# lpiccinelli-eth/UniDepth

Measured on NVIDIA H100. Metric: images/sec UniDepthV2.infer ViT-L/14 480x640, higher is better.
Workload: dtype f16 operands, f32 accumulate/residual

## Files before the change

include/udb.h:

```cpp
#ifndef UDB_H_
#define UDB_H_
#include <stddef.h>
#include <stdint.h>

#ifdef __cplusplus
extern "C" {
#endif

#define UDB_VERSION 1

int udb_version(void);

typedef struct udb_profile_entry_t {
  char name[48];
  float ms;
  double flops;
  double bytes;
} udb_profile_entry_t;
int udb_profile_begin(void* stream);
int udb_profile_end(udb_profile_entry_t* out, int32_t cap);
const char* udb_last_error(void);
int64_t udb_launch_count(void);

enum { UDB_A_MATRIX = 0, UDB_A_CONV3X3 = 1 };
// ... 16 lines not shown
  int32_t out_f32;
  void* out2;
  int32_t out2_leaky;
  int32_t act;
  int32_t store_mode;
  int64_t ldc;
  int32_t rows_per_group, group_stride, row_offset;
  int32_t resid_mod, resid_row_offset;
  int64_t ldr;
  int32_t ct_k, ct_cout, ct_h, ct_w, ct_pad;
  const float* head_w;
  float head_b, head_add;
  int32_t a_split_k;
  int32_t out_split;
  float* ln_stats_out;
  const float* ln_stats_in;
  const float* ln_c1;
  int32_t ln_parts, ln_part_cols;
  float ln_eps;
} udb_gemm_t;

int udb_gemm_f16(const udb_gemm_t* g, void* stream);
int udb_gemm_tma_epilogue_used(void);

typedef struct udb_conv_halo_t {
  const void* x;
  const void* w;
  const float* bias;
  int32_t B, H, W, C, cstride, coff, cout, act;
  void* out;
  int64_t ldc;
  const float* head_w;
  float head_b, head_add;
  float* head_out;
} udb_conv_halo_t;
int udb_conv3x3_halo_f16(const udb_conv_halo_t* c, void* stream);

typedef struct udb_attn_t {
  const void* q;
  const void* k;
  const void* v;
  void* out;
  int32_t B, heads, seq_q, seq_k, head_dim;
  int32_t ldq, ldk, ldv, ldo;
  int32_t q_col0, k_col0, v_col0, o_col0;
  float scale;
// ... 373 lines not shown
```

unidepth_b200/_cabi.py:

```python
from __future__ import annotations

import ctypes as C
import os

_HERE = os.path.dirname(os.path.abspath(__file__))
LIB_PATH = os.environ.get("UDB_LIB", os.path.join(_HERE, "libudb.so"))

A_MATRIX, A_CONV3X3 = 0, 1
ACT_NONE, ACT_GELU, ACT_LEAKY = 0, 1, 2
STORE_ROWS, STORE_CONVT, STORE_CONVTILE, STORE_HEAD = 0, 1, 2, 3
INTERP_BILINEAR, INTERP_BICUBIC = 0, 1
INTERP_MODES = {"bilinear": INTERP_BILINEAR, "bicubic": INTERP_BICUBIC}
CAM_NONE, CAM_PINHOLE, CAM_EUCM, CAM_SPHERICAL, CAM_OPENCV, CAM_FISHEYE624, CAM_MEI = range(7)
CAM_STRIDE = 20

vp, i32, i64, f32 = C.c_void_p, C.c_int32, C.c_int64, C.c_float


class Gemm(C.Structure):
    _fields_ = [
        ("a", vp), ("w", vp), ("M", i32), ("N", i32), ("K", i32), ("lda", i32), ("ldw", i32),
        ("a_mode", i32),
        ("conv_B", i32), ("conv_H", i32), ("conv_W", i32), ("conv_C", i32), ("conv_inH", i32),
        ("conv_inW", i32), ("conv_off", i32), ("conv_TH", i32), ("conv_TW", i32),
        ("conv_cstride", i32), ("conv_coff", i32),
        ("bias", vp), ("gamma", vp), ("resid", vp), ("resid_f32", i32), ("out", vp), ("out_f32", i32),
        ("out2", vp), ("out2_leaky", i32), ("act", i32), ("store_mode", i32), ("ldc", i64),
        ("rows_per_group", i32), ("group_stride", i32), ("row_offset", i32),
        ("resid_mod", i32), ("resid_row_offset", i32), ("ldr", i64),
        ("ct_k", i32), ("ct_cout", i32), ("ct_h", i32), ("ct_w", i32), ("ct_pad", i32),
        ("head_w", vp), ("head_b", f32), ("head_add", f32),
        ("a_split_k", i32), ("out_split", i32),
        ("ln_stats_out", vp), ("ln_stats_in", vp), ("ln_c1", vp), ("ln_parts", i32), ("ln_part_cols", i32), ("ln_eps", f32),
    ]


class ConvHalo(C.Structure):
    _fields_ = [
        ("x", vp), ("w", vp), ("bias", vp),
        ("B", i32), ("H", i32), ("W", i32), ("C", i32), ("cstride", i32), ("coff", i32), ("cout", i32), ("act", i32),
        ("out", vp), ("ldc", i64), ("head_w", vp), ("head_b", f32), ("head_add", f32), ("head_out", vp),
    ]


class Attn(C.Structure):
    _fields_ = [
        ("q", vp), ("k", vp), ("v", vp), ("out", vp),
        ("B", i32), ("heads", i32), ("seq_q", i32), ("seq_k", i32), ("head_dim", i32),
        ("ldq", i32), ("ldk", i32), ("ldv", i32), ("ldo", i32),
        ("q_col0", i32), ("k_col0", i32), ("v_col0", i32), ("o_col0", i32), ("scale", f32),
        ("split", i32), ("lo_off_q", i32), ("lo_off_k", i32), ("lo_off_v", i32), ("lo_off_o", i32),
    ]


class LayerNorm(C.Structure):
    _fields_ = [
        ("inp", vp), ("in_f32", i32), ("out", vp), ("out_f32", i32), ("weight", vp), ("bias", vp),
        ("rows", i32), ("dim", i32), ("ld_in", i64), ("ld_out", i64),
        ("rows_per_group", i32), ("group_stride", i32), ("row_offset", i32), ("eps", f32), ("dim_valid", i32),
# ... 138 lines not shown
METRIC_MAX_BLOCKS = 64
DM_AUC_BINS = 100
(DM_N, DM_D1, DM_D2, DM_D3, DM_TAU, DM_SQ, DM_SQLOG, DM_AREL, DM_SQREL, DM_LOG10, DM_LG, DM_LG2, DM_D1_SI, DM_TAU_SI,
 DM_AREL_SI, DM_PP, DM_P, DM_PG, DM_G, DM_AUC) = range(20)
DM_AREL_SSI, DM_D1_SSI, DM_TAU_SSI = DM_AUC + DM_AUC_BINS, DM_AUC + DM_AUC_BINS + 1, DM_AUC + DM_AUC_BINS + 2
DM_NACC = DM_TAU_SSI + 1
PM_MAX_THRESHOLDS = 1024


class ProfileEntry(C.Structure):
    _fields_ = [("name", C.c_char * 48), ("ms", f32), ("flops", C.c_double), ("bytes", C.c_double)]


DT_F16, DT_F32 = 0, 1

EXPORTS = {
    "udb_version": (i32, []),
    "udb_last_error": (C.c_char_p, []),
    "udb_launch_count": (i64, []),
    "udb_profile_begin": (i32, [vp]),
    "udb_profile_end": (i32, [C.POINTER(ProfileEntry), i32]),
    "udb_gemm_f16": (i32, [C.POINTER(Gemm), vp]),
    "udb_gemm_tma_epilogue_used": (i32, []),
    "udb_conv3x3_halo_f16": (i32, [C.POINTER(ConvHalo), vp]),
    "udb_attention_f16": (i32, [C.POINTER(Attn), vp]),
    "udb_layernorm": (i32, [C.POINTER(LayerNorm), vp]),
    "udb_preprocess_patchify": (i32, [C.POINTER(Preprocess), vp]),
    "udb_posembed_bicubic": (i32, [vp, i32, i32, vp, i32, i32, vp]),
    "udb_set_cls_rows": (i32, [vp, vp, vp, i32, i32, i32, vp]),
    "udb_set_cls_rows_ln": (i32, [vp, vp, vp, vp, vp, i32, i32, i32, i32, i32, vp]),
    "udb_small_linear_f32": (i32, [C.POINTER(SmallLinear), vp]),
    "udb_camera_attn4_f32": (i32, [vp, vp, vp, vp, i32, i32, i32, vp]),
    "udb_camera_intrinsics": (i32, [vp, i32, i32, i32, f32, i32, i32, vp, vp, vp, vp]),
    "udb_ray_embed": (i32, [C.POINTER(RayEmbed), vp]),
    "udb_upsample2x_nhwc_f16": (i32, [vp, vp, i32, i32, i32, i32, vp]),
    "udb_resize_ac_pad_nhwc_f16": (i32, [vp, vp, i32, i32, i32, i32, i32, i32, i32, vp]),
    "udb_reflect_pad1_nhwc_f16": (i32, [vp, vp, i32, i32, i32, i32, vp]),
    "udb_reflect_border_fill_nhwc_f16": (i32, [vp, i32, i32, i32, i32, vp]),
    "udb_postprocess": (i32, [C.POINTER(Postprocess), vp]),
    "udb_camera_adjust_k": (i32, [vp, i32, f32, i32, i32, vp, vp]),
    "udb_camera_rays": (i32, [i32, vp, i32, i32, i32, i32, i32, i32, i32, f32, vp, vp]),
    "udb_create": (i32, [C.POINTER(Config), C.POINTER(vp)]),
    "udb_destroy": (None, [vp]),
    "udb_set_weight": (i32, [vp, C.c_char_p, vp, C.POINTER(i64), i32, i32]),
    "udb_set_scalar": (i32, [vp, C.c_char_p, C.c_double]),
    "udb_geometry": (i32, [vp, i32, i32, i32, C.POINTER(Geometry)]),
# ... 82 lines not shown
```

unidepth_b200/csrc/gemm.cu:

```cuda
#include <stdlib.h>
#include <string.h>

#include "common.h"
#include "ptx.cuh"

namespace udb {

constexpr int BM = 128;
constexpr int BK = 64;
constexpr int kEpiWarps = 8;
constexpr int kTP = 36;
constexpr int kThreads = (kEpiWarps + 4) * 32;

struct GemmArgs {
  int M, N, K, num_kb;
  int tiles_m, tiles_n;
  int a_mode;
  int conv_B, conv_H, conv_W, conv_cpb , conv_off, conv_TH, conv_TW, conv_tx, conv_ty;
  const float* bias;
  const float* gamma;
  const void* resid;
  int resid_f32;
  void* out;
  int out_f32;
  __half* out2;
  int out2_leaky;
  int act;
  int store_mode;
  long long ldc, ldr;
  int rpg, gstride, roff;
  int resid_mod, resid_roff;
  int ct_k, ct_cout, ct_h, ct_w, ct_pad;
  int conv_coff;
  const float* head_w;
  float head_b, head_add;
  int a_wrap;
  int out_split;
  float* stats_out;
  const float* ln_stats;
  const float* ln_c1;
  int ln_parts, ln_part_cols;
  float ln_eps;
};

constexpr int kEpiBox = 64 * 32 * 4;

template <int BN, bool TMAE = false>
struct GemmCfg {
  static constexpr int kStages = TMAE ? (BN >= 192 ? 4 : (BN >= 128 ? 6 : 8))
                                      : (BN >= 256 ? 3 : (BN >= 192 ? 4 : (BN >= 128 ? 5 : 7)));
  static constexpr int kABytes = BM * BK * 2;
  static constexpr int kBBytes = BN * BK * 2;
  static constexpr int kStageBytes = kABytes + kBBytes;
  static constexpr int kStagingBytes = TMAE ? 2 * 2 * kEpiBox : kEpiWarps * (32 * kTP * 4 + 2 * 32 * 4);
  static constexpr int kSmemBytes = kStages * kStageBytes + kStagingBytes + 256 ;
  static_assert(kSmemBytes <= 232448, "shared memory per block");
  static_assert(2 * kStages + 4 <= 32, "barriers");
};

template <int N>
__device__ __forceinline__ void apply_act(const int act, float (&v)[N]) {
  if (act == UDB_ACT_GELU) {
#pragma unroll
    for (int j = 0; j < N; j += 2) gelu_erf_pair(v[j], v[j + 1]);
  } else if (act == UDB_ACT_LEAKY) {
#pragma unroll
    for (int j = 0; j < N; ++j) v[j] = leaky(v[j]);
  }
}

struct EpiWarp {
  float* T;
  float* Twg;
  uint32_t* roff_out;
  uint32_t* roff_res;
  int wg, wq, grp, lane, r_in_tile;
};

template <int BN, bool LNF>
__device__ __forceinline__ void epilogue_tile(const GemmArgs& p, const EpiWarp& w, const float (&acc)[BN / 2], const int mt,
                                              const int nt) {
  constexpr int kGroups = BN >= 64 ? 2 : 1;
  constexpr int kColsPerGrp = BN / kGroups;
  const int grp = w.grp, lane = w.lane, r_in_tile = w.r_in_tile;
  const bool active = grp < kGroups;
  float* T = w.T;
  uint32_t* roff_out = w.roff_out;
  uint32_t* roff_res = w.roff_res;
  bool valid = false;
  long long out_off = 0, res_off = 0;
  uint32_t vmask = 0;
  float ln_mean = 0.f, ln_rstd = 1.f;
  float st_pivot = 0.f, st_s1 = 0.f, st_s2 = 0.f;
  bool st_first = true;
  if (active) {

    const int m = mt * BM + r_in_tile;
    if (p.store_mode == UDB_STORE_CONVTILE || p.store_mode == UDB_STORE_HEAD) {
      const int per_img = p.conv_tx * p.conv_ty;
      const int b = mt / per_img;
      const int r = mt % per_img;
      const int y = (r / p.conv_tx) * p.conv_TH + r_in_tile / p.conv_TW;
      const int x = (r % p.conv_tx) * p.conv_TW + r_in_tile % p.conv_TW;
      valid = (b < p.conv_B) && (y < p.conv_H) && (x < p.conv_W);
// ... 30 lines not shown
        const float2 t = sp[q];
        m2 += t.y + (float)p.ln_part_cols * (t.x - ln_mean) * (t.x - ln_mean);
      }
      ln_rstd = rsqrtf(m2 / (float)(p.ln_parts * p.ln_part_cols) + p.ln_eps);
    }
  }
  const int frow = 16 * (w.wq & 1) + (lane >> 2), fcol = 2 * (lane & 3);
#pragma unroll
  for (int c = 0; c < kColsPerGrp; c += 32) {
    bar_sync(1 + w.wg, 128);
#pragma unroll
    for (int gi = 0; gi < kGroups; ++gi) {
      float* Tt = w.Twg + ((w.wq >> 1) | (gi << 1)) * 32 * kTP;
#pragma unroll
      for (int j = 0; j < 4; ++j) {
        const int f = ((gi * kColsPerGrp + c) / 8 + j) * 4;
        *reinterpret_cast<float2*>(Tt + frow * kTP + 8 * j + fcol) = make_float2(acc[f], acc[f + 1]);
        *reinterpret_cast<float2*>(Tt + (frow + 8) * kTP + 8 * j + fcol) = make_float2(acc[f + 2], acc[f + 3]);
      }
    }
    bar_sync(1 + w.wg, 128);
    if (!active) continue;
    const int col = grp * kColsPerGrp + c;
    const int n0 = nt * BN + col;
    float v[32];
#pragma unroll
    for (int j = 0; j < 32; j += 4) {
      const float4 t = *reinterpret_cast<const float4*>(T + lane * kTP + j);
      v[j] = t.x; v[j + 1] = t.y; v[j + 2] = t.z; v[j + 3] = t.w;
    }
    __syncwarp();
    if (n0 >= p.N) continue;
    if (LNF && p.ln_stats) {
      const float4* cp = reinterpret_cast<const float4*>(p.ln_c1 + n0);
      const float mr = ln_mean * ln_rstd;
#pragma unroll
      for (int j = 0; j < 8; ++j) {
        const float4 c4 = __ldg(cp + j);
        v[4 * j] = fmaf(v[4 * j], ln_rstd, -mr * c4.x);
        v[4 * j + 1] = fmaf(v[4 * j + 1], ln_rstd, -mr * c4.y);
        v[4 * j + 2] = fmaf(v[4 * j + 2], ln_rstd, -mr * c4.z);
        v[4 * j + 3] = fmaf(v[4 * j + 3], ln_rstd, -mr * c4.w);
      }
    }
    if (p.bias) {
      const float4* bp = reinterpret_cast<const float4*>(p.bias + n0);
#pragma unroll
// ... 117 lines not shown
    }
    if (p.out2) {
      if (p.out2_leaky) {
#pragma unroll
        for (int j = 0; j < 32; ++j) v[j] = leaky(v[j]);
        stage_rows(v);
      } else if (!p.out) {
        stage_rows(v);
      }
      __syncwarp();
      __half* op = p.out2 + c32 + l4;
      for_rows([&](int rr, bool ok) {
        const float4 t = *reinterpret_cast<const float4*>(T + rr * kTP + l4);
        if (ok) *reinterpret_cast<uint2*>(op + roff_out[rr]) = make_uint2(pack_half2(t.x, t.y), pack_half2(t.z, t.w));
      });
      __syncwarp();
    }
  }
  if (LNF && p.stats_out && active && valid && !st_first) {
    const float n = (float)kColsPerGrp;
    const float mean_p = st_pivot + st_s1 / n;
    const float m2_p = fmaxf(st_s2 - st_s1 * st_s1 / n, 0.f);
    const long long orow = out_off / p.ldc;
    reinterpret_cast<float2*>(p.stats_out)[orow * (p.tiles_n * kGroups) + nt * kGroups + grp] = make_float2(mean_p, m2_p);
  }
}

struct EpiTma {
  uint8_t* buf;
  uint64_t* full;
  uint64_t* empty;
  uint32_t chunk;
};

template <int BN>
__device__ __forceinline__ void epilogue_tile_tma(const GemmArgs& p, const CUtensorMap* tmC, EpiTma& e,
                                                  const float (&acc)[BN / 2], const int mt, const int nt, const int wg,
                                                  const int wq, const int lane) {
  const bool leader = wq == 0 && lane == 0;
  const int q = lane & 3, rr = lane >> 2;
  const bool has_res = p.resid != nullptr;
  const int row0 = mt * BM + 64 * wg;
#pragma unroll
  for (int c = 0; c < BN / 32; ++c, ++e.chunk) {
    const int b = e.chunk & 1;
    uint8_t* box = e.buf + (2 * b + wg) * kEpiBox;
    if (has_res) {
      mbar_wait(&e.full[b], (e.chunk >> 1) & 1);
    } else {
      if (leader) bulk_wait_read<1>();
      bar_sync(1 + wg, 128);
    }
    const int n0 = nt * BN + 32 * c;
    float v[16];
#pragma unroll
    for (int j = 0; j < 16; ++j) v[j] = acc[16 * c + j];
    if (p.bias) {
#pragma unroll
      for (int j = 0; j < 4; ++j) {
        const float2 b2 = __ldg(reinterpret_cast<const float2*>(p.bias + n0 + 8 * j + 2 * q));
        v[4 * j] += b2.x; v[4 * j + 1] += b2.y; v[4 * j + 2] += b2.x; v[4 * j + 3] += b2.y;
      }
    }
    apply_act(p.act, v);
    if (p.gamma) {
#pragma unroll
      for (int j = 0; j < 4; ++j) {
        const float2 g2 = __ldg(reinterpret_cast<const float2*>(p.gamma + n0 + 8 * j + 2 * q));
        v[4 * j] *= g2.x; v[4 * j + 1] *= g2.y; v[4 * j + 2] *= g2.x; v[4 * j + 3] *= g2.y;
      }
    }
    if (p.out_f32) {
#pragma unroll
      for (int j = 0; j < 4; ++j) {
#pragma unroll
        for (int h = 0; h < 2; ++h) {
// ... 11 lines not shown
#pragma unroll
      for (int j = 0; j < 4; ++j) {
#pragma unroll
        for (int h = 0; h < 2; ++h) {
          const int r = 16 * wq + rr + 8 * h;
          *reinterpret_cast<uint32_t*>(box + r * 64 + ((j ^ ((r >> 1) & 3)) << 4) + 4 * q) =
              pack_half2(v[4 * j + 2 * h], v[4 * j + 2 * h + 1]);
        }
      }
    }
    fence_proxy_async_smem();
    bar_sync(1 + wg, 128);
    if (leader) {
      if (row0 < p.M) tma_store_2d(tmC, box, n0, row0);
      bulk_commit();
      if (has_res) {
        bulk_wait_read<0>();
        mbar_arrive(&e.empty[b]);
      }
    }
  }
}

template <int BN, bool LNF, bool TMAE>
__global__ void __launch_bounds__(kThreads, 1)
gemm_f16_kernel(const __grid_constant__ CUtensorMap tmA, const __grid_constant__ CUtensorMap tmB,
                const __grid_constant__ CUtensorMap tmC, const __grid_constant__ CUtensorMap tmR, const GemmArgs p) {
  static_assert(!(TMAE && LNF), "the TMA epilogue carries no fused-LayerNorm code");
  using Cfg = GemmCfg<BN, TMAE>;
  constexpr int kStages = Cfg::kStages;
  extern __shared__ __align__(1024) uint8_t smem[];
  uint8_t* sA = smem;
  uint8_t* sB = smem + kStages * Cfg::kABytes;
  uint8_t* staging = smem + kStages * Cfg::kStageBytes;
  uint64_t* bars = reinterpret_cast<uint64_t*>(staging + Cfg::kStagingBytes);
  uint64_t* full_bar = bars;
  uint64_t* empty_bar = bars + kStages;
  uint64_t* epi_full = bars + 2 * kStages;
  uint64_t* epi_empty = epi_full + 2;

  const int warp = threadIdx.x >> 5;
  const int lane = threadIdx.x & 31;
  pdl_launch_dependents();

  if (threadIdx.x == 0) {
    if (smem_u32(smem) & 1023) __trap();
    prefetch_tmap(&tmA);
    prefetch_tmap(&tmB);
    for (int i = 0; i < kStages; ++i) {
      mbar_init(&full_bar[i], 1);
      mbar_init(&empty_bar[i], kEpiWarps);
    }
    if constexpr (TMAE) {
      prefetch_tmap(&tmC);
      if (p.resid) prefetch_tmap(&tmR);
      for (int i = 0; i < 2; ++i) {
        mbar_init(&epi_full[i], 1);
        mbar_init(&epi_empty[i], 2);
      }
    }
    fence_barrier_init();
  }
  __syncthreads();
  pdl_wait();

  const int num_tiles = p.tiles_m * p.tiles_n;

  if (warp >= kEpiWarps) {
    setmaxnreg_dec<40>();
    if constexpr (TMAE) {
      if (warp == kEpiWarps + 1 && p.resid) {
        const bool elected = elect_one();
        uint32_t chunk = 0;
        for (int tile = blockIdx.x; tile < num_tiles; tile += gridDim.x) {
          const int mt = tile / p.tiles_n;
          const int nt = tile % p.tiles_n;
          for (int c = 0; c < BN / 32; ++c, ++chunk) {
            const int b = chunk & 1;
            mbar_wait(&epi_empty[b], ((chunk >> 1) & 1) ^ 1);
            if (elected) {
              mbar_arrive_expect_tx(&epi_full[b], 2 * kEpiBox);
              tma_load_2d(staging + 2 * b * kEpiBox, &tmR, &epi_full[b], nt * BN + 32 * c, mt * BM);
            }
            __syncwarp();
          }
        }
      }
    }
    if (warp != kEpiWarps) return;
    const bool elected = elect_one();
    int stage = 0;
    uint32_t phase = 0;
    for (int tile = blockIdx.x; tile < num_tiles; tile += gridDim.x) {
      const int mt = tile / p.tiles_n;
      const int nt = tile % p.tiles_n;
      int cb = 0, cy = 0, cx = 0;
      if (p.a_mode == UDB_A_CONV3X3) {
        const int per_img = p.conv_tx * p.conv_ty;
        cb = mt / per_img;
        const int r = mt % per_img;
        cy = (r / p.conv_tx) * p.conv_TH + p.conv_off;
        cx = (r % p.conv_tx) * p.conv_TW + p.conv_off;
      }
      for (int kb = 0; kb < p.num_kb; ++kb) {
        mbar_wait(&empty_bar[stage], phase ^ 1);
        if (elected) {
          mbar_arrive_expect_tx(&full_bar[stage], Cfg::kStageBytes);
          if (p.a_mode == UDB_A_CONV3X3) {
            const int tap = kb / p.conv_cpb;
            const int c0 = p.conv_coff + (kb % p.conv_cpb) * BK;
            tma_load_4d(sA + stage * Cfg::kABytes, &tmA, &full_bar[stage], c0, cx + tap % 3, cy + tap / 3, cb);
          } else {
            int ka = kb * BK;
            if (p.a_wrap && ka >= p.a_wrap) ka -= p.a_wrap;
            tma_load_2d(sA + stage * Cfg::kABytes, &tmA, &full_bar[stage], ka, mt * BM);
          }
          tma_load_2d(sB + stage * Cfg::kBBytes, &tmB, &full_bar[stage], kb * BK, nt * BN);
        }
        __syncwarp();
        if (++stage == kStages) {
          stage = 0;
          phase ^= 1;
        }
      }
    }
  } else {
    setmaxnreg_inc<232>();
    const int wg = warp >> 2, wq = warp & 3;
    float* Twg = reinterpret_cast<float*>(staging) + wg * 4 * 32 * kTP;
    uint32_t* roff = reinterpret_cast<uint32_t*>(staging + kEpiWarps * 32 * kTP * 4) + warp * 64;
    const EpiWarp ctx{Twg + wq * 32 * kTP, Twg, roff, roff + 32, wg, wq, wq >> 1, lane, 64 * wg + 32 * (wq & 1) + lane};
    EpiTma etma{staging, epi_full, epi_empty, 0};
    float acc[BN / 2];
#pragma unroll
    for (int i = 0; i < BN / 2; ++i) acc[i] = 0.f;
    int stage = 0;
    uint32_t phase = 0;
    for (int tile = blockIdx.x; tile < num_tiles; tile += gridDim.x) {
      const int mt = tile / p.tiles_n;
      const int nt = tile % p.tiles_n;
      int prev = -1;
      for (int kb = 0; kb < p.num_kb; ++kb) {
        mbar_wait(&full_bar[stage], phase);
        const uint64_t da = gmma_desc_sw128(smem_u32(sA + stage * Cfg::kABytes + wg * 64 * 128), 16, 1024);
        const uint64_t db = gmma_desc_sw128(smem_u32(sB + stage * Cfg::kBBytes), 16, 1024);
        wgmma_fence();
#pragma unroll
        for (int k = 0; k < BK / 16; ++k) WgmmaSS<BN>::run(acc, da + 2 * k, db + 2 * k, (kb | k) != 0 ? 1u : 0u);
        wgmma_commit();
        wgmma_wait<1>();
        if (prev >= 0 && lane == 0) mbar_arrive(&empty_bar[prev]);
        prev = stage;
        if (++stage == kStages) {
          stage = 0;
          phase ^= 1;
        }
      }
      wgmma_wait<0>();
      wgmma_fence_regs(acc);
      if (prev >= 0 && lane == 0) mbar_arrive(&empty_bar[prev]);
      if constexpr (TMAE) epilogue_tile_tma<BN>(p, &tmC, etma, acc, mt, nt, wg, wq, lane);
      else epilogue_tile<BN, LNF>(p, ctx, acc, mt, nt);
    }
    if constexpr (TMAE) {
      if (wq == 0 && lane == 0) bulk_wait<0>();
    }
  }
}

template <int BN, bool LNF, bool TMAE>
static int launch_gemm(const CUtensorMap& tmA, const CUtensorMap& tmB, const CUtensorMap& tmC, const CUtensorMap& tmR,
                       const GemmArgs& a, cudaStream_t st) {
  using Cfg = GemmCfg<BN, TMAE>;
  static std::atomic<uint64_t> attr_mask{0};
  if (first_on_device(attr_mask)) {
    cudaError_t e = cudaFuncSetAttribute(gemm_f16_kernel<BN, LNF, TMAE>, cudaFuncAttributeMaxDynamicSharedMemorySize,
                                         Cfg::kSmemBytes);
    if (e != cudaSuccess) {
      set_error("gemm: cudaFuncSetAttribute(%d B smem): %s", Cfg::kSmemBytes, cudaGetErrorString(e));
      return 1;
    }
  }
  const int tiles = a.tiles_m * a.tiles_n;
  const int grid = tiles < num_sms() ? tiles : num_sms();
  cudaError_t e = launch_ex(gemm_f16_kernel<BN, LNF, TMAE>, dim3(grid), dim3(kThreads), Cfg::kSmemBytes, st, 1, tmA, tmB, tmC,
                            tmR, a);
  if (e != cudaSuccess) {
    set_error("gemm_f16_kernel launch: %s", cudaGetErrorString(e));
    return 1;
  }
  return check_launch("gemm_f16_kernel");
}

static bool aligned(const void* p, uintptr_t bytes) { return (reinterpret_cast<uintptr_t>(p) & (bytes - 1)) == 0; }

static int check_gemm_layout(const udb_gemm_t* g) {
  const int sm = g->store_mode;
  if (g->M < 1 || g->N < 1 || g->K < 1) { set_error("udb_gemm_f16: M=%d N=%d K=%d must be >= 1", g->M, g->N, g->K); return 1; }
  if (sm < UDB_STORE_ROWS || sm > UDB_STORE_HEAD) { set_error("udb_gemm_f16: unknown store_mode %d", sm); return 1; }
  const long long ldr = g->ldr > 0 ? g->ldr : g->ldc;
  if (sm == UDB_STORE_HEAD) {
    if (!g->out || !g->out_f32 || !aligned(g->out, 4)) { set_error("udb_gemm_f16: HEAD store needs a 4-byte aligned f32 `out`"); return 1; }
    if (!g->head_w || !aligned(g->head_w, 16)) { set_error("udb_gemm_f16: `head_w` must be non-null and 16-byte aligned"); return 1; }
  } else {
    if (g->out && !aligned(g->out, g->out_f32 ? 16 : 8)) {
      set_error("udb_gemm_f16: `out` %p must be %d-byte aligned", g->out, g->out_f32 ? 16 : 8); return 1;
    }
    if (g->out2 && !aligned(g->out2, 8)) { set_error("udb_gemm_f16: `out2` %p must be 8-byte aligned", g->out2); return 1; }
    if (g->resid && !aligned(g->resid, g->resid_f32 ? 16 : 8)) {
// ... 58 lines not shown

  if (g->a_mode == UDB_A_CONV3X3) {
    const int pad = g->conv_off == 0 ? 2 : (g->conv_off == -1 ? 0 : -1);
    if (pad < 0) { set_error("udb_gemm_f16: `conv_off`=%d must be 0 (prepadded) or -1 (zero padding)", g->conv_off); return 1; }
    if (g->conv_inH != g->conv_H + pad || g->conv_inW != g->conv_W + pad) {
      set_error("udb_gemm_f16: `conv_inH`x`conv_inW` = %dx%d must be %dx%d for conv_off %d", g->conv_inH, g->conv_inW, g->conv_H + pad,
                g->conv_W + pad, g->conv_off);
      return 1;
    }
  }
  return 0;
}

static bool tma_epilogue_ok(const udb_gemm_t* g) {
  const char* env = getenv("UDB_GEMM_TMA_EPILOGUE");
  if (env && atoi(env) == 0) return false;
  if (g->store_mode != UDB_STORE_ROWS || g->a_mode != UDB_A_MATRIX || g->rows_per_group > 0 || g->resid_mod > 0) return false;
  if (g->out_split || g->out2 || g->ln_stats_out || g->ln_stats_in || !g->out) return false;
  if (!aligned(g->out, 16) || (g->ldc * (g->out_f32 ? 4 : 2)) % 16) return false;
  const long long ldr = g->ldr > 0 ? g->ldr : g->ldc;
  return !g->resid || (g->resid_f32 && g->out_f32 && aligned(g->resid, 16) && (ldr * 4) % 16 == 0);
}

static thread_local int g_last_tma_epilogue = 0;

}

extern "C" int udb_gemm_tma_epilogue_used(void) { return udb::g_last_tma_epilogue; }

extern "C" int udb_gemm_f16(const udb_gemm_t* g, void* stream) {
  using namespace udb;
  if (!g || !g->a || !g->w) { set_error("udb_gemm_f16: null operand"); return 1; }
  if (g->N % 32 != 0) { set_error("udb_gemm_f16: N=%d must be a multiple of 32", g->N); return 1; }
  if (check_gemm_layout(g)) return 1;
  GemmArgs a{};
  a.M = g->M; a.N = g->N; a.K = g->K;
  a.num_kb = (g->K + BK - 1) / BK;
  a.a_mode = g->a_mode;
  a.bias = g->bias; a.gamma = g->gamma; a.resid = g->resid; a.resid_f32 = g->resid_f32;
  a.out = g->out; a.out_f32 = g->out_f32; a.out2 = reinterpret_cast<__half*>(g->out2); a.out2_leaky = g->out2_leaky;
  a.act = g->act; a.store_mode = g->store_mode;
  a.ldc = g->ldc; a.ldr = g->ldr > 0 ? g->ldr : g->ldc;
  a.rpg = g->rows_per_group; a.gstride = g->group_stride; a.roff = g->row_offset;
  a.resid_mod = g->resid_mod; a.resid_roff = g->resid_row_offset;
  a.ct_k = g->ct_k; a.ct_cout = g->ct_cout; a.ct_h = g->ct_h; a.ct_w = g->ct_w; a.ct_pad = g->ct_pad;
  a.conv_coff = g->conv_coff;
  a.head_w = g->head_w; a.head_b = g->head_b; a.head_add = g->head_add;
  a.a_wrap = 0;
  a.out_split = g->out_split;
  if (g->a_split_k > 0) {
    if (g->a_mode != UDB_A_MATRIX || g->a_split_k % BK || g->K != 3 * g->a_split_k || g->lda < 2 * g->a_split_k) {
      set_error("udb_gemm_f16: split operands need a_mode MATRIX, K1 %% 64 == 0, K == 3*K1, lda >= 2*K1 (K1=%d K=%d lda=%d)",
                g->a_split_k, g->K, g->lda);
      return 1;
    }
    a.a_wrap = 2 * g->a_split_k;
  }
  a.stats_out = g->ln_stats_out; a.ln_stats = g->ln_stats_in; a.ln_c1 = g->ln_c1; a.ln_eps = g->ln_eps;
  a.ln_parts = g->ln_parts; a.ln_part_cols = g->ln_part_cols;
  if ((g->ln_stats_out || g->ln_stats_in) && g->store_mode != UDB_STORE_ROWS) {
    set_error("udb_gemm_f16: fused LayerNorm statistics need the ROWS store"); return 1;
  }
  if (g->ln_stats_in && (!g->ln_c1 || g->ln_parts <= 0 || g->ln_part_cols <= 0 || g->rows_per_group > 0)) {
    set_error("udb_gemm_f16: ln_stats_in needs ln_c1, ln_parts, ln_part_cols and an identity row map"); return 1;
  }
  if (g->out_split && (g->out_f32 || !g->out || g->store_mode != UDB_STORE_ROWS)) {
    set_error("udb_gemm_f16: out_split needs an f16 `out` with the ROWS store"); return 1;
  }

  int bn;
  if (g->store_mode == UDB_STORE_HEAD) {
    if (g->N != 32) { set_error("udb_gemm_f16: HEAD store needs N == 32"); return 1; }
    bn = 32;
  } else if (g->N % 256 == 0) bn = 256;
  else if (g->N % 192 == 0) bn = 192;
  else if (g->N % 128 == 0) bn = 128;
  else if (g->N % 64 == 0) bn = 64;
  else bn = 32;
  if (g->store_mode == UDB_STORE_CONVT && (g->ct_cout % 32) != 0) {
    set_error("udb_gemm_f16: CONVT needs Cout %% 32 == 0"); return 1;
  }
  a.tiles_n = (g->N + bn - 1) / bn;
  if (g->ln_stats_out) {
    const int groups = bn >= 64 ? 2 : 1;
    if (g->N % bn || g->ln_parts != a.tiles_n * groups || g->ln_part_cols != bn / groups) {
      set_error("udb_gemm_f16: ln_stats_out with N=%d runs as %d parts of %d columns (caller said %d x %d)", g->N, a.tiles_n * groups,
                bn / groups, g->ln_parts, g->ln_part_cols);
      return 1;
    }
  }

  CUtensorMap tmA, tmB;
  if (g->a_mode == UDB_A_CONV3X3) {
    if (g->conv_C % BK != 0 || g->K != 9 * g->conv_C) {
      set_error("udb_gemm_f16: conv3x3 needs C %% 64 == 0 and K == 9*C (C=%d K=%d)", g->conv_C, g->K);
      return 1;
    }
    if (g->store_mode != UDB_STORE_CONVTILE && g->store_mode != UDB_STORE_HEAD) {
      set_error("udb_gemm_f16: conv3x3 operand needs a CONVTILE or HEAD store"); return 1;
    }
    const int TH = g->conv_TH > 0 ? g->conv_TH : 8, TW = g->conv_TW > 0 ? g->conv_TW : 16;
    if (TH * TW != BM) { set_error("udb_gemm_f16: conv tile %dx%d != 128 pixels", TH, TW); return 1; }
    a.conv_B = g->conv_B; a.conv_H = g->conv_H; a.conv_W = g->conv_W; a.conv_cpb = g->conv_C / BK; a.conv_off = g->conv_off;
    a.conv_TH = TH; a.conv_TW = TW;
    a.conv_tx = (g->conv_W + TW - 1) / TW; a.conv_ty = (g->conv_H + TH - 1) / TH;
    a.tiles_m = g->conv_B * a.conv_tx * a.conv_ty;
    a.M = a.tiles_m * BM;
    const uint64_t cs = g->conv_cstride > 0 ? g->conv_cstride : g->conv_C;
    if ((uint64_t)g->conv_coff + g->conv_C > cs || (g->conv_coff % 8)) {
      set_error("udb_gemm_f16: bad conv channel slice (off %d, C %d, stride %d)", g->conv_coff, g->conv_C, (int)cs);
      return 1;
    }
    const uint64_t dims[4] = {cs, (uint64_t)g->conv_inW, (uint64_t)g->conv_inH, (uint64_t)g->conv_B};
    const uint64_t str[3] = {cs * 2, (uint64_t)g->conv_inW * cs * 2, (uint64_t)g->conv_inH * g->conv_inW * cs * 2};
    const uint32_t box[4] = {(uint32_t)BK, (uint32_t)TW, (uint32_t)TH, 1};
    if (make_tmap_f16(&tmA, g->a, 4, dims, str, box, true)) return 1;
  } else {
    a.tiles_m = (g->M + BM - 1) / BM;
    if (g->store_mode == UDB_STORE_CONVTILE || g->store_mode == UDB_STORE_HEAD) {
      set_error("udb_gemm_f16: tile store modes need a_mode == CONV3X3"); return 1;
    }
    const uint64_t dims[2] = {(uint64_t)(g->a_split_k > 0 ? 2 * g->a_split_k : g->K), (uint64_t)g->M};
    const uint64_t str[1] = {(uint64_t)g->lda * 2};
    const uint32_t box[2] = {(uint32_t)BK, (uint32_t)BM};
    if (make_tmap_f16(&tmA, g->a, 2, dims, str, box, true)) return 1;
  }
  {
    const uint64_t dims[2] = {(uint64_t)g->K, (uint64_t)g->N};
    const uint64_t str[1] = {(uint64_t)g->ldw * 2};
    const uint32_t box[2] = {(uint32_t)BK, (uint32_t)bn};
    if (make_tmap_f16(&tmB, g->w, 2, dims, str, box, true)) return 1;
  }
  const bool tmae = tma_epilogue_ok(g);
  CUtensorMap tmC, tmR;
  memset(&tmC, 0, sizeof(tmC));
  memset(&tmR, 0, sizeof(tmR));
  if (tmae) {
    const uint64_t dims[2] = {(uint64_t)g->N, (uint64_t)g->M};
    const uint64_t str_c[1] = {(uint64_t)g->ldc * (g->out_f32 ? 4 : 2)};
    const uint32_t box_c[2] = {32, 64};
    if (make_tmap(&tmC, g->out, 2, dims, str_c, box_c, g->out_f32 ? CU_TENSOR_MAP_DATA_TYPE_FLOAT32 : CU_TENSOR_MAP_DATA_TYPE_FLOAT16,
                  g->out_f32 ? CU_TENSOR_MAP_SWIZZLE_128B : CU_TENSOR_MAP_SWIZZLE_64B))
      return 1;
    if (g->resid) {
      const uint64_t str_r[1] = {(uint64_t)a.ldr * 4};
      const uint32_t box_r[2] = {32, BM};
      if (make_tmap(&tmR, g->resid, 2, dims, str_r, box_r, CU_TENSOR_MAP_DATA_TYPE_FLOAT32, CU_TENSOR_MAP_SWIZZLE_128B)) return 1;
    }
  }
  g_last_tma_epilogue = tmae ? 1 : 0;
  cudaStream_t st = reinterpret_cast<cudaStream_t>(stream);
  note_work(2.0 * a.M * (double)g->N * g->K,
            2.0 * ((double)a.M * (g->a_mode == UDB_A_CONV3X3 ? g->conv_C : (g->a_split_k ? 2 * g->a_split_k : g->K)) + (double)g->N * g->K) +
                (double)a.M * g->N * ((g->out ? (g->out_f32 ? 4 : 2) : 0) + (g->out2 ? 2 : 0) + (g->resid ? (g->resid_f32 ? 4 : 2) : 0)));
  const bool lnf = g->ln_stats_out || g->ln_stats_in;
  if (lnf) {
    switch (bn) {
      case 256: return launch_gemm<256, true, false>(tmA, tmB, tmC, tmR, a, st);
      case 192: return launch_gemm<192, true, false>(tmA, tmB, tmC, tmR, a, st);
      case 128: return launch_gemm<128, true, false>(tmA, tmB, tmC, tmR, a, st);
      case 64: return launch_gemm<64, true, false>(tmA, tmB, tmC, tmR, a, st);
      default: return launch_gemm<32, true, false>(tmA, tmB, tmC, tmR, a, st);
    }
  }
  if (tmae) {
    switch (bn) {
      case 256: return launch_gemm<256, false, true>(tmA, tmB, tmC, tmR, a, st);
      case 192: return launch_gemm<192, false, true>(tmA, tmB, tmC, tmR, a, st);
      case 128: return launch_gemm<128, false, true>(tmA, tmB, tmC, tmR, a, st);
      case 64: return launch_gemm<64, false, true>(tmA, tmB, tmC, tmR, a, st);
      default: return launch_gemm<32, false, true>(tmA, tmB, tmC, tmR, a, st);
    }
  }
  switch (bn) {
    case 256: return launch_gemm<256, false, false>(tmA, tmB, tmC, tmR, a, st);
    case 192: return launch_gemm<192, false, false>(tmA, tmB, tmC, tmR, a, st);
    case 128: return launch_gemm<128, false, false>(tmA, tmB, tmC, tmR, a, st);
    case 64: return launch_gemm<64, false, false>(tmA, tmB, tmC, tmR, a, st);
    default: return launch_gemm<32, false, false>(tmA, tmB, tmC, tmR, a, st);
  }
}
```

Baseline: 222.4.

## Split last-wave GEMM tiles into narrow N units to balance persistent scheduling

```diff
diff --git a/include/udb.h b/include/udb.h
--- a/include/udb.h
+++ b/include/udb.h
@@ -62,6 +62,13 @@
 
 int udb_gemm_f16(const udb_gemm_t* g, void* stream);
 int udb_gemm_tma_epilogue_used(void);
+
+typedef struct udb_gemm_plan_t {
+  int32_t bn, tiles_m, tiles_n, grid, full, units, width;
+} udb_gemm_plan_t;
+int udb_gemm_plan(const udb_gemm_t* g, int32_t num_sms, udb_gemm_plan_t* plan);
+int udb_gemm_plan_unit(const udb_gemm_plan_t* plan, int32_t unit, int32_t* mt, int32_t* n0, int32_t* width);
+int udb_gemm_last_units(int32_t* full, int32_t* narrow, int32_t* width);
 
 typedef struct udb_conv_halo_t {
   const void* x;
diff --git a/unidepth_b200/_cabi.py b/unidepth_b200/_cabi.py
--- a/unidepth_b200/_cabi.py
+++ b/unidepth_b200/_cabi.py
@@ -35,6 +35,10 @@
     ]
 
 
+class GemmPlan(C.Structure):
+    _fields_ = [("bn", i32), ("tiles_m", i32), ("tiles_n", i32), ("grid", i32), ("full", i32), ("units", i32), ("width", i32)]
+
+
 class ConvHalo(C.Structure):
     _fields_ = [
         ("x", vp), ("w", vp), ("bias", vp),
@@ -219,6 +223,9 @@
     "udb_profile_end": (i32, [C.POINTER(ProfileEntry), i32]),
     "udb_gemm_f16": (i32, [C.POINTER(Gemm), vp]),
     "udb_gemm_tma_epilogue_used": (i32, []),
+    "udb_gemm_plan": (i32, [C.POINTER(Gemm), i32, C.POINTER(GemmPlan)]),
+    "udb_gemm_plan_unit": (i32, [C.POINTER(GemmPlan), i32, C.POINTER(i32), C.POINTER(i32), C.POINTER(i32)]),
+    "udb_gemm_last_units": (i32, [C.POINTER(i32), C.POINTER(i32), C.POINTER(i32)]),
     "udb_conv3x3_halo_f16": (i32, [C.POINTER(ConvHalo), vp]),
     "udb_attention_f16": (i32, [C.POINTER(Attn), vp]),
     "udb_layernorm": (i32, [C.POINTER(LayerNorm), vp]),
diff --git a/unidepth_b200/csrc/gemm.cu b/unidepth_b200/csrc/gemm.cu
--- a/unidepth_b200/csrc/gemm.cu
+++ b/unidepth_b200/csrc/gemm.cu
@@ -1,5 +1,7 @@
 #include <stdlib.h>
 #include <string.h>
+
+#include <type_traits>
 
 #include "common.h"
 #include "ptx.cuh"
@@ -41,7 +43,19 @@
   const float* ln_c1;
   int ln_parts, ln_part_cols;
   float ln_eps;
+  int units, units_full;
 };
+
+__host__ __device__ constexpr int tail_width(int bn) { return bn >= 128 ? 64 : 32; }
+
+struct GemmUnit {
+  int mt, n0, width;
+};
+__host__ __device__ __forceinline__ GemmUnit gemm_unit(int u, int tiles_n, int bn, int full, int w) {
+  if (u < full) return {u / tiles_n, (u % tiles_n) * bn, bn};
+  const int per = bn / w, r = u - full, tile = full + r / per;
+  return {tile / tiles_n, (tile % tiles_n) * bn + (r % per) * w, w};
+}
 
 constexpr int kEpiBox = 64 * 32 * 4;
 
@@ -79,7 +93,7 @@
 
 template <int BN, bool LNF>
 __device__ __forceinline__ void epilogue_tile(const GemmArgs& p, const EpiWarp& w, const float (&acc)[BN / 2], const int mt,
-                                              const int nt) {
+                                              const int nb) {
   constexpr int kGroups = BN >= 64 ? 2 : 1;
   constexpr int kColsPerGrp = BN / kGroups;
   const int grp = w.grp, lane = w.lane, r_in_tile = w.r_in_tile;
@@ -156,7 +170,7 @@
     bar_sync(1 + w.wg, 128);
     if (!active) continue;
     const int col = grp * kColsPerGrp + c;
-    const int n0 = nt * BN + col;
+    const int n0 = nb + col;
     float v[32];
 #pragma unroll
     for (int j = 0; j < 32; j += 4) {
@@ -320,7 +334,7 @@
     const float mean_p = st_pivot + st_s1 / n;
     const float m2_p = fmaxf(st_s2 - st_s1 * st_s1 / n, 0.f);
     const long long orow = out_off / p.ldc;
-    reinterpret_cast<float2*>(p.stats_out)[orow * (p.tiles_n * kGroups) + nt * kGroups + grp] = make_float2(mean_p, m2_p);
+    reinterpret_cast<float2*>(p.stats_out)[orow * (p.tiles_n * kGroups) + (nb / BN) * kGroups + grp] = make_float2(mean_p, m2_p);
   }
 }
 
@@ -333,7 +347,7 @@
 
 template <int BN>
 __device__ __forceinline__ void epilogue_tile_tma(const GemmArgs& p, const CUtensorMap* tmC, EpiTma& e,
-                                                  const float (&acc)[BN / 2], const int mt, const int nt, const int wg,
+                                                  const float (&acc)[BN / 2], const int mt, const int nb, const int wg,
                                                   const int wq, const int lane) {
   const bool leader = wq == 0 && lane == 0;
   const int q = lane & 3, rr = lane >> 2;
@@ -349,7 +363,7 @@
       if (leader) bulk_wait_read<1>();
       bar_sync(1 + wg, 128);
     }
-    const int n0 = nt * BN + 32 * c;
+    const int n0 = nb + 32 * c;
     float v[16];
 #pragma unroll
     for (int j = 0; j < 16; ++j) v[j] = acc[16 * c + j];
@@ -407,16 +421,25 @@
   }
 }
 
-template <int BN, bool LNF, bool TMAE>
+template <int BN, bool LNF, bool TMAE, bool SPLIT>
 __global__ void __launch_bounds__(kThreads, 1)
 gemm_f16_kernel(const __grid_constant__ CUtensorMap tmA, const __grid_constant__ CUtensorMap tmB,
-                const __grid_constant__ CUtensorMap tmC, const __grid_constant__ CUtensorMap tmR, const GemmArgs p) {
+                const __grid_constant__ CUtensorMap tmBn, const __grid_constant__ CUtensorMap tmC,
+                const __grid_constant__ CUtensorMap tmR, const GemmArgs p) {
   static_assert(!(TMAE && LNF), "the TMA epilogue carries no fused-LayerNorm code");
   using Cfg = GemmCfg<BN, TMAE>;
   constexpr int kStages = Cfg::kStages;
+  static_assert(!SPLIT || (!LNF && tail_width(BN) < BN), "no narrow units for this instantiation");
+  constexpr int kTW = SPLIT ? tail_width(BN) : BN;
+  constexpr int kNBBytes = kTW * BK * 2;
+  constexpr int kNK = SPLIT && Cfg::kBBytes >= Cfg::kABytes + 2 * kNBBytes ? 2 : 1;
   extern __shared__ __align__(1024) uint8_t smem[];
   uint8_t* sA = smem;
   uint8_t* sB = smem + kStages * Cfg::kABytes;
+  auto stage_a = [&](int s, int i) { return i == 0 ? sA + s * Cfg::kABytes : sB + s * Cfg::kBBytes; };
+  auto stage_b = [&](int s, int i, bool narrow) {
+    return sB + s * Cfg::kBBytes + (kNK == 2 && narrow ? Cfg::kABytes + i * kNBBytes : 0);
+  };
   uint8_t* staging = smem + kStages * Cfg::kStageBytes;
   uint64_t* bars = reinterpret_cast<uint64_t*>(staging + Cfg::kStagingBytes);
   uint64_t* full_bar = bars;
@@ -432,6 +455,7 @@
     if (smem_u32(smem) & 1023) __trap();
     prefetch_tmap(&tmA);
     prefetch_tmap(&tmB);
+    if (SPLIT) prefetch_tmap(&tmBn);
     for (int i = 0; i < kStages; ++i) {
       mbar_init(&full_bar[i], 1);
       mbar_init(&empty_bar[i], kEpiWarps);
@@ -449,23 +473,20 @@
   __syncthreads();
   pdl_wait();
 
-  const int num_tiles = p.tiles_m * p.tiles_n;
-
   if (warp >= kEpiWarps) {
     setmaxnreg_dec<40>();
     if constexpr (TMAE) {
       if (warp == kEpiWarps + 1 && p.resid) {
         const bool elected = elect_one();
         uint32_t chunk = 0;
-        for (int tile = blockIdx.x; tile < num_tiles; tile += gridDim.x) {
-          const int mt = tile / p.tiles_n;
-          const int nt = tile % p.tiles_n;
-          for (int c = 0; c < BN / 32; ++c, ++chunk) {
+        for (int u = blockIdx.x; u < p.units; u += gridDim.x) {
+          const GemmUnit t = gemm_unit(u, p.tiles_n, BN, p.units_full, kTW);
+          for (int c = 0; c < t.width / 32; ++c, ++chunk) {
             const int b = chunk & 1;
             mbar_wait(&epi_empty[b], ((chunk >> 1) & 1) ^ 1);
             if (elected) {
               mbar_arrive_expect_tx(&epi_full[b], 2 * kEpiBox);
-              tma_load_2d(staging + 2 * b * kEpiBox, &tmR, &epi_full[b], nt * BN + 32 * c, mt * BM);
+              tma_load_2d(staging + 2 * b * kEpiBox, &tmR, &epi_full[b], t.n0 + 32 * c, t.mt * BM);
             }
             __syncwarp();
           }
@@ -476,9 +497,12 @@
     const bool elected = elect_one();
     int stage = 0;
     uint32_t phase = 0;
-    for (int tile = blockIdx.x; tile < num_tiles; tile += gridDim.x) {
-      const int mt = tile / p.tiles_n;
-      const int nt = tile % p.tiles_n;
+    for (int u = blockIdx.x; u < p.units; u += gridDim.x) {
+      const GemmUnit t = gemm_unit(u, p.tiles_n, BN, p.units_full, kTW);
+      const int mt = t.mt;
+      const bool narrow = SPLIT && t.width != BN;
+      const CUtensorMap* tmW = narrow ? &tmBn : &tmB;
+      const int kpb = narrow ? kNK : 1;
       int cb = 0, cy = 0, cx = 0;
       if (p.a_mode == UDB_A_CONV3X3) {
         const int per_img = p.conv_tx * p.conv_ty;
@@ -487,20 +511,24 @@
         cy = (r / p.conv_tx) * p.conv_TH + p.conv_off;
         cx = (r % p.conv_tx) * p.conv_TW + p.conv_off;
       }
-      for (int kb = 0; kb < p.num_kb; ++kb) {
+      for (int kb0 = 0; kb0 < p.num_kb; kb0 += kpb) {
         mbar_wait(&empty_bar[stage], phase ^ 1);
         if (elected) {
-          mbar_arrive_expect_tx(&full_bar[stage], Cfg::kStageBytes);
-          if (p.a_mode == UDB_A_CONV3X3) {
-            const int tap = kb / p.conv_cpb;
-            const int c0 = p.conv_coff + (kb % p.conv_cpb) * BK;
-            tma_load_4d(sA + stage * Cfg::kABytes, &tmA, &full_bar[stage], c0, cx + tap % 3, cy + tap / 3, cb);
-          } else {
-            int ka = kb * BK;
-            if (p.a_wrap && ka >= p.a_wrap) ka -= p.a_wrap;
-            tma_load_2d(sA + stage * Cfg::kABytes, &tmA, &full_bar[stage], ka, mt * BM);
+          const int nk = kpb == 1 || p.num_kb - kb0 >= kpb ? kpb : p.num_kb - kb0;
+          mbar_arrive_expect_tx(&full_bar[stage], nk * (Cfg::kABytes + t.width * BK * 2));
+          for (int i = 0; i < nk; ++i) {
+            const int kb = kb0 + i;
+            if (p.a_mode == UDB_A_CONV3X3) {
+              const int tap = kb / p.conv_cpb;
+              const int c0 = p.conv_coff + (kb % p.conv_cpb) * BK;
+              tma_load_4d(stage_a(stage, i), &tmA, &full_bar[stage], c0, cx + tap % 3, cy + tap / 3, cb);
+            } else {
+              int ka = kb * BK;
+              if (p.a_wrap && ka >= p.a_wrap) ka -= p.a_wrap;
+              tma_load_2d(stage_a(stage, i), &tmA, &full_bar[stage], ka, mt * BM);
+            }
+            tma_load_2d(stage_b(stage, i, narrow), tmW, &full_bar[stage], kb * BK, t.n0);
           }
-          tma_load_2d(sB + stage * Cfg::kBBytes, &tmB, &full_bar[stage], kb * BK, nt * BN);
         }
         __syncwarp();
         if (++stage == kStages) {
@@ -521,18 +549,24 @@
     for (int i = 0; i < BN / 2; ++i) acc[i] = 0.f;
     int stage = 0;
     uint32_t phase = 0;
-    for (int tile = blockIdx.x; tile < num_tiles; tile += gridDim.x) {
-      const int mt = tile / p.tiles_n;
-      const int nt = tile % p.tiles_n;
+    auto run_unit = [&](auto width, const GemmUnit& t) {
+      constexpr int W = decltype(width)::value;
+      float(&accw)[W / 2] = *reinterpret_cast<float(*)[W / 2]>(acc);
+      constexpr int KPB = W != BN ? kNK : 1;
       int prev = -1;
-      for (int kb = 0; kb < p.num_kb; ++kb) {
+      for (int kb0 = 0; kb0 < p.num_kb; kb0 += KPB) {
         mbar_wait(&full_bar[stage], phase);
-        const uint64_t da = gmma_desc_sw128(smem_u32(sA + stage * Cfg::kABytes + wg * 64 * 128), 16, 1024);
-        const uint64_t db = gmma_desc_sw128(smem_u32(sB + stage * Cfg::kBBytes), 16, 1024);
-        wgmma_fence();
-#pragma unroll
-        for (int k = 0; k < BK / 16; ++k) WgmmaSS<BN>::run(acc, da + 2 * k, db + 2 * k, (kb | k) != 0 ? 1u : 0u);
-        wgmma_commit();
+#pragma unroll
+        for (int i = 0; i < KPB; ++i) {
+          const int kb = kb0 + i;
+          if (i > 0 && kb >= p.num_kb) break;
+          const uint64_t da = gmma_desc_sw128(smem_u32(stage_a(stage, i) + wg * 64 * 128), 16, 1024);
+          const uint64_t db = gmma_desc_sw128(smem_u32(stage_b(stage, i, W != BN)), 16, 1024);
+          wgmma_fence();
+#pragma unroll
+          for (int k = 0; k < BK / 16; ++k) WgmmaSS<W>::run(accw, da + 2 * k, db + 2 * k, (kb | k) != 0 ? 1u : 0u);
+          wgmma_commit();
+        }
         wgmma_wait<1>();
         if (prev >= 0 && lane == 0) mbar_arrive(&empty_bar[prev]);
         prev = stage;
@@ -542,10 +576,20 @@
         }
       }
       wgmma_wait<0>();
-      wgmma_fence_regs(acc);
+      wgmma_fence_regs(accw);
       if (prev >= 0 && lane == 0) mbar_arrive(&empty_bar[prev]);
-      if constexpr (TMAE) epilogue_tile_tma<BN>(p, &tmC, etma, acc, mt, nt, wg, wq, lane);
-      else epilogue_tile<BN, LNF>(p, ctx, acc, mt, nt);
+      if constexpr (TMAE) epilogue_tile_tma<W>(p, &tmC, etma, accw, t.mt, t.n0, wg, wq, lane);
+      else epilogue_tile<W, LNF>(p, ctx, accw, t.mt, t.n0);
+    };
+    for (int u = blockIdx.x; u < p.units; u += gridDim.x) {
+      const GemmUnit t = gemm_unit(u, p.tiles_n, BN, p.units_full, kTW);
+      if constexpr (kTW < BN) {
+        if (t.width != BN) {
+          run_unit(std::integral_constant<int, kTW>{}, t);
+          continue;
+        }
+      }
+      run_unit(std::integral_constant<int, BN>{}, t);
     }
     if constexpr (TMAE) {
       if (wq == 0 && lane == 0) bulk_wait<0>();
@@ -553,23 +597,21 @@
   }
 }
 
-template <int BN, bool LNF, bool TMAE>
-static int launch_gemm(const CUtensorMap& tmA, const CUtensorMap& tmB, const CUtensorMap& tmC, const CUtensorMap& tmR,
-                       const GemmArgs& a, cudaStream_t st) {
+template <int BN, bool LNF, bool TMAE, bool SPLIT = false>
+static int launch_gemm(const CUtensorMap& tmA, const CUtensorMap& tmB, const CUtensorMap& tmBn, const CUtensorMap& tmC,
+                       const CUtensorMap& tmR, const GemmArgs& a, int grid, cudaStream_t st) {
   using Cfg = GemmCfg<BN, TMAE>;
   static std::atomic<uint64_t> attr_mask{0};
   if (first_on_device(attr_mask)) {
-    cudaError_t e = cudaFuncSetAttribute(gemm_f16_kernel<BN, LNF, TMAE>, cudaFuncAttributeMaxDynamicSharedMemorySize,
+    cudaError_t e = cudaFuncSetAttribute(gemm_f16_kernel<BN, LNF, TMAE, SPLIT>, cudaFuncAttributeMaxDynamicSharedMemorySize,
                                          Cfg::kSmemBytes);
     if (e != cudaSuccess) {
       set_error("gemm: cudaFuncSetAttribute(%d B smem): %s", Cfg::kSmemBytes, cudaGetErrorString(e));
       return 1;
     }
   }
-  const int tiles = a.tiles_m * a.tiles_n;
-  const int grid = tiles < num_sms() ? tiles : num_sms();
-  cudaError_t e = launch_ex(gemm_f16_kernel<BN, LNF, TMAE>, dim3(grid), dim3(kThreads), Cfg::kSmemBytes, st, 1, tmA, tmB, tmC,
-                            tmR, a);
+  cudaError_t e = launch_ex(gemm_f16_kernel<BN, LNF, TMAE, SPLIT>, dim3(grid), dim3(kThreads), Cfg::kSmemBytes, st, 1, tmA, tmB, tmBn,
+                            tmC, tmR, a);
   if (e != cudaSuccess) {
     set_error("gemm_f16_kernel launch: %s", cudaGetErrorString(e));
     return 1;
@@ -674,11 +716,70 @@
   return !g->resid || (g->resid_f32 && g->out_f32 && aligned(g->resid, 16) && (ldr * 4) % 16 == 0);
 }
 
+static int plan_gemm(const udb_gemm_t* g, int sms, udb_gemm_plan_t* pl) {
+  if (g->M < 1 || g->N < 1 || g->K < 1 || g->N % 32 || sms < 1) {
+    set_error("udb_gemm: M=%d N=%d K=%d (N %% 32 == 0) on %d SMs", g->M, g->N, g->K, sms);
+    return 1;
+  }
+  int bn;
+  if (g->store_mode == UDB_STORE_HEAD) {
+    if (g->N != 32) { set_error("udb_gemm_f16: HEAD store needs N == 32"); return 1; }
+    bn = 32;
+  } else if (g->N % 256 == 0) bn = 256;
+  else if (g->N % 192 == 0) bn = 192;
+  else if (g->N % 128 == 0) bn = 128;
+  else if (g->N % 64 == 0) bn = 64;
+  else bn = 32;
+  int tiles_m;
+  if (g->a_mode == UDB_A_CONV3X3) {
+    const int TH = g->conv_TH > 0 ? g->conv_TH : 8, TW = g->conv_TW > 0 ? g->conv_TW : 16;
+    tiles_m = g->conv_B * ((g->conv_W + TW - 1) / TW) * ((g->conv_H + TH - 1) / TH);
+  } else {
+    tiles_m = (g->M + BM - 1) / BM;
+  }
+  const int tiles_n = (g->N + bn - 1) / bn, tiles = tiles_m * tiles_n;
+  const int grid = tiles < sms ? tiles : sms;
+  *pl = udb_gemm_plan_t{bn, tiles_m, tiles_n, grid, tiles, tiles, bn};
+  const char* env = getenv("UDB_GEMM_TAIL_SPLIT");
+  const int w = tail_width(bn);
+  if ((env && atoi(env) == 0) || w == bn || g->ln_stats_out || g->ln_stats_in || g->store_mode == UDB_STORE_HEAD) return 0;
+  const int full = (tiles - 1) / grid * grid, rem = tiles - full;
+  if (rem * (bn / w) <= grid / 4) {
+    pl->full = full;
+    pl->units = full + rem * (bn / w);
+    pl->width = w;
+  }
+  return 0;
+}
+
 static thread_local int g_last_tma_epilogue = 0;
+static thread_local udb_gemm_plan_t g_last_plan{};
 
 }
 
 extern "C" int udb_gemm_tma_epilogue_used(void) { return udb::g_last_tma_epilogue; }
+
+extern "C" int udb_gemm_last_units(int32_t* full, int32_t* narrow, int32_t* width) {
+  const udb_gemm_plan_t& pl = udb::g_last_plan;
+  if (full) *full = pl.full;
+  if (narrow) *narrow = pl.units - pl.full;
+  if (width) *width = pl.units > pl.full ? pl.width : 0;
+  return 0;
+}
+
+extern "C" int udb_gemm_plan(const udb_gemm_t* g, int32_t num_sms, udb_gemm_plan_t* plan) {
+  if (!g || !plan) { udb::set_error("udb_gemm_plan: null argument"); return 1; }
+  return udb::plan_gemm(g, num_sms, plan);
+}
+
+extern "C" int udb_gemm_plan_unit(const udb_gemm_plan_t* plan, int32_t unit, int32_t* mt, int32_t* n0, int32_t* width) {
+  if (!plan || unit < 0 || unit >= plan->units) { udb::set_error("udb_gemm_plan_unit: no unit %d", unit); return 1; }
+  const udb::GemmUnit t = udb::gemm_unit(unit, plan->tiles_n, plan->bn, plan->full, plan->width);
+  *mt = t.mt;
+  *n0 = t.n0;
+  *width = t.width;
+  return 0;
+}
 
 extern "C" int udb_gemm_f16(const udb_gemm_t* g, void* stream) {
   using namespace udb;
@@ -720,19 +821,16 @@
     set_error("udb_gemm_f16: out_split needs an f16 `out` with the ROWS store"); return 1;
   }
 
-  int bn;
-  if (g->store_mode == UDB_STORE_HEAD) {
-    if (g->N != 32) { set_error("udb_gemm_f16: HEAD store needs N == 32"); return 1; }
-    bn = 32;
-  } else if (g->N % 256 == 0) bn = 256;
-  else if (g->N % 192 == 0) bn = 192;
-  else if (g->N % 128 == 0) bn = 128;
-  else if (g->N % 64 == 0) bn = 64;
-  else bn = 32;
+  udb_gemm_plan_t pl;
+  if (plan_gemm(g, num_sms(), &pl)) return 1;
+  const int bn = pl.bn;
   if (g->store_mode == UDB_STORE_CONVT && (g->ct_cout % 32) != 0) {
     set_error("udb_gemm_f16: CONVT needs Cout %% 32 == 0"); return 1;
   }
-  a.tiles_n = (g->N + bn - 1) / bn;
+  a.tiles_m = pl.tiles_m;
+  a.tiles_n = pl.tiles_n;
+  a.units = pl.units;
+  a.units_full = pl.full;
   if (g->ln_stats_out) {
     const int groups = bn >= 64 ? 2 : 1;
     if (g->N % bn || g->ln_parts != a.tiles_n * groups || g->ln_part_cols != bn / groups) {
@@ -742,7 +840,7 @@
     }
   }
 
-  CUtensorMap tmA, tmB;
+  CUtensorMap tmA, tmB, tmBn;
   if (g->a_mode == UDB_A_CONV3X3) {
     if (g->conv_C % BK != 0 || g->K != 9 * g->conv_C) {
       set_error("udb_gemm_f16: conv3x3 needs C %% 64 == 0 and K == 9*C (C=%d K=%d)", g->conv_C, g->K);
@@ -756,7 +854,6 @@
     a.conv_B = g->conv_B; a.conv_H = g->conv_H; a.conv_W = g->conv_W; a.conv_cpb = g->conv_C / BK; a.conv_off = g->conv_off;
     a.conv_TH = TH; a.conv_TW = TW;
     a.conv_tx = (g->conv_W + TW - 1) / TW; a.conv_ty = (g->conv_H + TH - 1) / TH;
-    a.tiles_m = g->conv_B * a.conv_tx * a.conv_ty;
     a.M = a.tiles_m * BM;
     const uint64_t cs = g->conv_cstride > 0 ? g->conv_cstride : g->conv_C;
     if ((uint64_t)g->conv_coff + g->conv_C > cs || (g->conv_coff % 8)) {
@@ -768,7 +865,6 @@
     const uint32_t box[4] = {(uint32_t)BK, (uint32_t)TW, (uint32_t)TH, 1};
     if (make_tmap_f16(&tmA, g->a, 4, dims, str, box, true)) return 1;
   } else {
-    a.tiles_m = (g->M + BM - 1) / BM;
     if (g->store_mode == UDB_STORE_CONVTILE || g->store_mode == UDB_STORE_HEAD) {
       set_error("udb_gemm_f16: tile store modes need a_mode == CONV3X3"); return 1;
     }
@@ -782,6 +878,9 @@
     const uint64_t str[1] = {(uint64_t)g->ldw * 2};
     const uint32_t box[2] = {(uint32_t)BK, (uint32_t)bn};
     if (make_tmap_f16(&tmB, g->w, 2, dims, str, box, true)) return 1;
+    memset(&tmBn, 0, sizeof(tmBn));
+    const uint32_t box_n[2] = {(uint32_t)BK, (uint32_t)pl.width};
+    if (pl.units > pl.full && make_tmap_f16(&tmBn, g->w, 2, dims, str, box_n, true)) return 1;
   }
   const bool tmae = tma_epilogue_ok(g);
   CUtensorMap tmC, tmR;
@@ -801,6 +900,7 @@
     }
   }
   g_last_tma_epilogue = tmae ? 1 : 0;
+  g_last_plan = pl;
   cudaStream_t st = reinterpret_cast<cudaStream_t>(stream);
   note_work(2.0 * a.M * (double)g->N * g->K,
             2.0 * ((double)a.M * (g->a_mode == UDB_A_CONV3X3 ? g->conv_C : (g->a_split_k ? 2 * g->a_split_k : g->K)) + (double)g->N * g->K) +
@@ -808,27 +908,39 @@
   const bool lnf = g->ln_stats_out || g->ln_stats_in;
   if (lnf) {
     switch (bn) {
-      case 256: return launch_gemm<256, true, false>(tmA, tmB, tmC, tmR, a, st);
-      case 192: return launch_gemm<192, true, false>(tmA, tmB, tmC, tmR, a, st);
-      case 128: return launch_gemm<128, true, false>(tmA, tmB, tmC, tmR, a, st);
-      case 64: return launch_gemm<64, true, false>(tmA, tmB, tmC, tmR, a, st);
-      default: return launch_gemm<32, true, false>(tmA, tmB, tmC, tmR, a, st);
+      case 256: return launch_gemm<256, true, false>(tmA, tmB, tmBn, tmC, tmR, a, pl.grid, st);
+      case 192: return launch_gemm<192, true, false>(tmA, tmB, tmBn, tmC, tmR, a, pl.grid, st);
+      case 128: return launch_gemm<128, true, false>(tmA, tmB, tmBn, tmC, tmR, a, pl.grid, st);
+      case 64: return launch_gemm<64, true, false>(tmA, tmB, tmBn, tmC, tmR, a, pl.grid, st);
+      default: return launch_gemm<32, true, false>(tmA, tmB, tmBn, tmC, tmR, a, pl.grid, st);
+    }
+  }
+  if (pl.units > pl.full) {
+    switch (bn * 2 + tmae) {
+      case 513: return launch_gemm<256, false, true, true>(tmA, tmB, tmBn, tmC, tmR, a, pl.grid, st);
+      case 512: return launch_gemm<256, false, false, true>(tmA, tmB, tmBn, tmC, tmR, a, pl.grid, st);
+      case 385: return launch_gemm<192, false, true, true>(tmA, tmB, tmBn, tmC, tmR, a, pl.grid, st);
+      case 384: return launch_gemm<192, false, false, true>(tmA, tmB, tmBn, tmC, tmR, a, pl.grid, st);
+      case 257: return launch_gemm<128, false, true, true>(tmA, tmB, tmBn, tmC, tmR, a, pl.grid, st);
+      case 256: return launch_gemm<128, false, false, true>(tmA, tmB, tmBn, tmC, tmR, a, pl.grid, st);
+      case 129: return launch_gemm<64, false, true, true>(tmA, tmB, tmBn, tmC, tmR, a, pl.grid, st);
+      default: return launch_gemm<64, false, false, true>(tmA, tmB, tmBn, tmC, tmR, a, pl.grid, st);
     }
   }
   if (tmae) {
     switch (bn) {
-      case 256: return launch_gemm<256, false, true>(tmA, tmB, tmC, tmR, a, st);
-      case 192: return launch_gemm<192, false, true>(tmA, tmB, tmC, tmR, a, st);
-      case 128: return launch_gemm<128, false, true>(tmA, tmB, tmC, tmR, a, st);
-      case 64: return launch_gemm<64, false, true>(tmA, tmB, tmC, tmR, a, st);
-      default: return launch_gemm<32, false, true>(tmA, tmB, tmC, tmR, a, st);
+      case 256: return launch_gemm<256, false, true>(tmA, tmB, tmBn, tmC, tmR, a, pl.grid, st);
+      case 192: return launch_gemm<192, false, true>(tmA, tmB, tmBn, tmC, tmR, a, pl.grid, st);
+      case 128: return launch_gemm<128, false, true>(tmA, tmB, tmBn, tmC, tmR, a, pl.grid, st);
+      case 64: return launch_gemm<64, false, true>(tmA, tmB, tmBn, tmC, tmR, a, pl.grid, st);
+      default: return launch_gemm<32, false, true>(tmA, tmB, tmBn, tmC, tmR, a, pl.grid, st);
     }
   }
   switch (bn) {
-    case 256: return launch_gemm<256, false, false>(tmA, tmB, tmC, tmR, a, st);
-    case 192: return launch_gemm<192, false, false>(tmA, tmB, tmC, tmR, a, st);
-    case 128: return launch_gemm<128, false, false>(tmA, tmB, tmC, tmR, a, st);
-    case 64: return launch_gemm<64, false, false>(tmA, tmB, tmC, tmR, a, st);
-    default: return launch_gemm<32, false, false>(tmA, tmB, tmC, tmR, a, st);
-  }
-}
+    case 256: return launch_gemm<256, false, false>(tmA, tmB, tmBn, tmC, tmR, a, pl.grid, st);
+    case 192: return launch_gemm<192, false, false>(tmA, tmB, tmBn, tmC, tmR, a, pl.grid, st);
+    case 128: return launch_gemm<128, false, false>(tmA, tmB, tmBn, tmC, tmR, a, pl.grid, st);
+    case 64: return launch_gemm<64, false, false>(tmA, tmB, tmBn, tmC, tmR, a, pl.grid, st);
+    default: return launch_gemm<32, false, false>(tmA, tmB, tmBn, tmC, tmR, a, pl.grid, st);
+  }
+}
```

Result: no change. 223.0 (median of 6 runs) (+0.3%).
